# StarsX/RayTracedGGX

Hardware: AMD Instinct MI355X
Metric: Mrays/s + ms/frame, bunny 1920x1080 1spp+denoise, 1/2/4/8 GPUs (higher is better)
Workload: dtype f32; 1 GPU; configs[1]: bunny.obj + rnl_cross env, 1920x1080, 1spp GGX reflection + full denoise chain (refl H,V; diff H,V, shared-memory variant; temporal; tone map), all-metal default materials, dt=1/60; parallelism=row strips x1, history_apron_rows=18, history_overreach_rows=0, setup_priming_frames=256, trace_workgroup_waves=12

## Files before the change

### raytracedggx_amd/csrc/raytrace.hip

```cpp
#include <cstring>
#include "rt_queue.h"
#include "rt_traverse.h"

namespace rt {

#define RT_PI 3.1415926535897f
#define RT_SGPR(v) ((uint32_t)__builtin_amdgcn_readfirstlane((int)(v)))

struct EnvRef { const uint2* __restrict__ texels; uint32_t size, mips; const uint32_t* __restrict__ mipOffset; };

RT_DEV void cubeFaceUV(f3 d, int& face, float& u, float& v) {
  const float ax = fabsf(d.x), ay = fabsf(d.y), az = fabsf(d.z);
  if (ax >= ay && ax >= az) { face = d.x >= 0.0f ? 0 : 1; u = (d.x >= 0.0f ? -d.z : d.z) / ax; v = -d.y / ax; }
  else if (ay >= az) { face = d.y >= 0.0f ? 2 : 3; u = d.x / ay; v = (d.y >= 0.0f ? d.z : -d.z) / ay; }
  else { face = d.z >= 0.0f ? 4 : 5; u = (d.z >= 0.0f ? d.x : -d.x) / az; v = -d.y / az; }
}
RT_DEV f3 cubeFaceDir(int face, float u, float v) {
  switch (face) {
    case 0: return mk3(1.0f, -v, -u);
    case 1: return mk3(-1.0f, -v, u);
    case 2: return mk3(u, 1.0f, v);
    case 3: return mk3(u, -1.0f, -v);
    case 4: return mk3(u, -v, 1.0f);
    default: return mk3(-u, -v, -1.0f);
  }
}
template <bool MIP0 = false>
RT_DEV f3 cubeTexel(const EnvRef& e, uint32_t mip, int face, int x, int y) {
  const int s = (int)((e.size >> mip) ? (e.size >> mip) : 1u);
  if (x < 0 || y < 0 || x >= s || y >= s) {
    const float u = ((float)x + 0.5f) / (float)s * 2.0f - 1.0f, v = ((float)y + 0.5f) / (float)s * 2.0f - 1.0f;
    float uu, vv; cubeFaceUV(cubeFaceDir(face, u, v), face, uu, vv);
    x = (int)floorf((uu * 0.5f + 0.5f) * (float)s); y = (int)floorf((vv * 0.5f + 0.5f) * (float)s);
    x = min(max(x, 0), s - 1); y = min(max(y, 0), s - 1);
  }
  const uint2 t = e.texels[(MIP0 ? 0u : e.mipOffset[mip]) + (uint32_t)face * (uint32_t)(s * s) + (uint32_t)(y * s + x)];
  return mk3(f16ToF32(t.x & 0xFFFFu), f16ToF32(t.x >> 16), f16ToF32(t.y & 0xFFFFu));
}
template <bool MIP0 = false>
RT_DEV f3 cubeBilinear(const EnvRef& e, uint32_t mip, int face, float u, float v) {
  const int s = (int)((e.size >> mip) ? (e.size >> mip) : 1u);
  const float x = (u * 0.5f + 0.5f) * (float)s - 0.5f, y = (v * 0.5f + 0.5f) * (float)s - 0.5f;
  const float x0 = floorf(x), y0 = floorf(y);
  const float fx = x - x0, fy = y - y0;
  const int ix = (int)x0, iy = (int)y0;
  const float w00 = (1.0f - fx) * (1.0f - fy), w10 = fx * (1.0f - fy), w01 = (1.0f - fx) * fy, w11 = fx * fy;
  const f3 c00 = cubeTexel<MIP0>(e, mip, face, ix, iy), c10 = cubeTexel<MIP0>(e, mip, face, ix + 1, iy);
  const f3 c01 = cubeTexel<MIP0>(e, mip, face, ix, iy + 1), c11 = cubeTexel<MIP0>(e, mip, face, ix + 1, iy + 1);
  return ((c00 * w00 + c10 * w10) + c01 * w01) + c11 * w11;
}
RT_DEV f3 environmentLevel0(const EnvRef& e, f3 dir) {
  int face; float u, v; cubeFaceUV(dir, face, u, v);
  return cubeBilinear<true>(e, 0u, face, u, v);
}
__device__ __noinline__ f3 environment(EnvRef e, f3 dir, float level) {
  int face; float u, v; cubeFaceUV(dir, face, u, v);
  const float maxLevel = (float)(e.mips - 1);
  const float l = fminf(fmaxf(level, 0.0f), maxLevel);
  const float l0 = floorf(l), fl = l - l0;
  const uint32_t m0 = (uint32_t)l0, m1 = min(m0 + 1, e.mips - 1);
  const f3 a = cubeBilinear(e, m0, face, u, v);
  if (fl == 0.0f) return a;
  const f3 b = cubeBilinear(e, m1, face, u, v);
  return a * (1.0f - fl) + b * fl;
}

RT_DEV f3 evaluateSHIrradiance(const float* __restrict__ sh, f3 norm) {
  const float c1 = 0.42904276540489171563379376569857f, c2 = 0.51166335397324424423977581244463f;
  const float c3 = 0.24770795610037568833406429782001f, c4 = 0.88622692545275801364908374167057f;
  const float x = -norm.x, y = -norm.y, z = norm.z;
#define SHL(i) mk3(sh[3 * (i)], sh[3 * (i) + 1], sh[3 * (i) + 2])
  f3 irr = (c1 * (x * x - y * y)) * SHL(8);
  irr = irr + (c3 * (3.0f * z * z - 1.0f)) * SHL(6);
  irr = irr + c4 * SHL(0);
  irr = irr + (2.0f * c1) * ((SHL(4) * x * y + SHL(7) * x * z) + SHL(5) * y * z);
  irr = irr + (2.0f * c2) * ((SHL(3) * x + SHL(1) * y) + SHL(2) * z);
#undef SHL
  return mk3(fmaxf(0.0f, irr.x), fmaxf(0.0f, irr.y), fmaxf(0.0f, irr.z));
}

RT_DEV f2 getUV(f3 n, f3 p, f3 scl) {
  f2 uv; uv.x = fabsf(n.x) * p.y * scl.y; uv.y = fabsf(n.x) * p.z * scl.z;
  uv.x += fabsf(n.y) * p.z * scl.z; uv.y += fabsf(n.y) * p.x * scl.x;
  uv.x += fabsf(n.z) * p.x * scl.x; uv.y += fabsf(n.z) * p.y * scl.y;
  uv.x = uv.x * 0.5f + 0.5f; uv.y = uv.y * 0.5f + 0.5f;
  return uv;
}
RT_DEV f2 getRoughMetal(const RtggxCBMaterial& mat, uint32_t inst, f2 uv) {
  float rough = mat.RoughMetals[inst][0];
  if (inst == 0) {
    const uint32_t px = ftou(uv.x * 5.0f) & 1u, py = ftou(uv.y * 5.0f) & 1u;
    rough = (px ^ py) ? rough * 0.25f : rough;
  }
  f2 r; r.x = rough; r.y = mat.RoughMetals[inst][1];
  return r;
}

RT_DEV float visSmith(float roughness, float NoV, float NoL) {
  const float a = roughness * roughness, a2 = a * a;
  const float v = NoV + sqrtf(NoV * (NoV - NoV * a2) + a2);
  const float l = NoL + sqrtf(NoL * (NoL - NoL * a2) + a2);
  return 1.0f / (v * l);
}
RT_DEV f3 fSchlick(f3 spec, float VoH) {
  const float x = 1.0f - VoH, x2 = x * x;
  const float fc = (x2 * x2) * x;
  const float s = saturatef(50.0f * spec.y) * fc;
  return mk3(s + (1.0f - fc) * spec.x, s + (1.0f - fc) * spec.y, s + (1.0f - fc) * spec.z);
// ... 23 lines not shown
  const f3 xAxis = normalize3(cross3(up, n));
  const f3 yAxis = cross3(n, xAxis);
  return (xAxis * l.x + yAxis * l.y) + n * l.z;
}
RT_DEV f3 vndfHalfVector(f3 n, f3 v, float alpha, float cosPhi, float sinPhi, float u) {
  const f3 up = fabsf(n.y) < 0.999f ? mk3(0.0f, 1.0f, 0.0f) : mk3(1.0f, 0.0f, 0.0f);
  const f3 xAxis = normalize3(cross3(up, n));
  const f3 yAxis = cross3(n, xAxis);
  const f3 ve = mk3(dot3(v, xAxis), dot3(v, yAxis), dot3(v, n));
  const f3 vh = normalize3(mk3(alpha * ve.x, alpha * ve.y, ve.z));
  const float lensq = vh.x * vh.x + vh.y * vh.y;
  const f3 t1v = lensq > 0.0f ? mk3(-vh.y, vh.x, 0.0f) * (1.0f / sqrtf(lensq)) : mk3(1.0f, 0.0f, 0.0f);
  const f3 t2v = cross3(vh, t1v);
  const float r = sqrtf(u);
  const float t1 = r * cosPhi;
  float t2 = r * sinPhi;
  const float sw = 0.5f * (1.0f + vh.z);
  t2 = (1.0f - sw) * sqrtf(1.0f - t1 * t1) + sw * t2;
  const f3 nh = (t1 * t1v + t2 * t2v) + sqrtf(fmaxf(0.0f, (1.0f - t1 * t1) - t2 * t2)) * vh;
  const f3 hl = normalize3(mk3(alpha * nh.x, alpha * nh.y, fmaxf(0.0f, nh.z)));
  return (xAxis * hl.x + yAxis * hl.y) + n * hl.z;
}
RT_DEV f3 reflectionHalfVector(bool vndf, f3 N, f3 V, float a, float cosPhi, float sinPhi, float xiY) {
  if (vndf) return vndfHalfVector(N, V, a, cosPhi, sinPhi, xiY);
  const float cosTheta = sqrtf((1.0f - xiY) / (1.0f + (a * a - 1.0f) * xiY));
  const float sinTheta = sqrtf(1.0f - cosTheta * cosTheta);
  return localToWorld(N, mk3(cosPhi * sinTheta, sinPhi * sinTheta, cosTheta));
}
RT_DEV f3 reflectionWeight(bool vndf, f3 N, f3 V, f3 Hh, float NoL, f2 rghMtl, f3 color) {
  const float a = rghMtl.x * rghMtl.x;
  const f3 f0 = mk3(lerpf(0.04f, color.x, rghMtl.y), lerpf(0.04f, color.y, rghMtl.y), lerpf(0.04f, color.z, rghMtl.y));
  const float NoV = saturatef(dot3(N, V));
  const float VoH = saturatef(dot3(V, Hh));
  const f3 F = fSchlick(f0, VoH);
  const float vis = visSmith(rghMtl.x, NoV, NoL);
  const float NoH = saturatef(dot3(N, Hh));
  const float k = 4.0f * VoH / NoH;
  f3 w = mk3(((NoL * F.x) * vis) * k, ((NoL * F.y) * vis) * k, ((NoL * F.z) * vis) * k);
  if (vndf) {
    const float a2 = a * a;
    const float g1l = (2.0f * NoL) / (NoL + sqrtf(NoL * (NoL - NoL * a2) + a2));
    w = mk3(F.x * g1l, F.y * g1l, F.z * g1l);
  }
  return w;
}
RT_DEV f3 diffuseDirection(f3 N, float cosPhi, float sinPhi, float xiY) {
  const float cosTheta = 1.0f - 2.0f * xiY;
  const float sinTheta = sqrtf(1.0f - cosTheta * cosTheta);
  return normalize3(N + mk3(cosPhi * sinTheta, sinPhi * sinTheta, cosTheta));
}
struct Tri3 { f3 pos[3], nrm[3]; };
RT_DEV Tri3 getVertices(const float4* __restrict__ fat, uint32_t prim) {
  const float4* p = fat + 5 * (size_t)prim;
  const float4 a = p[0], b = p[1], c = p[2], d = p[3], e = p[4];
  Tri3 v;
  v.pos[0] = mk3(a.x, a.y, a.z); v.nrm[0] = mk3(a.w, b.x, b.y);
  v.pos[1] = mk3(b.z, b.w, c.x); v.nrm[1] = mk3(c.y, c.z, c.w);
  v.pos[2] = mk3(d.x, d.y, d.z); v.nrm[2] = mk3(d.w, e.x, e.y);
  return v;
}
struct Attrib { f3 Pos, Nrm; f2 UV; };
RT_DEV Attrib interpAttrib(const Tri3& v, float b1, float b2) {
  const float w0 = 1.0f - (b1 + b2);
  Attrib a;
  a.Pos = (w0 * v.pos[0] + b1 * v.pos[1]) + b2 * v.pos[2];
  a.Nrm = (w0 * v.nrm[0] + b1 * v.nrm[1]) + b2 * v.nrm[2];
  a.UV = getUV(a.Nrm, a.Pos, mk3(1.0f, 0.2f, 1.0f));
  return a;
}
RT_DEV f2 calcBarycentrics(const f4 p[3], f2 ndc) {
  const f3 invW = mk3(1.0f / p[0].w, 1.0f / p[1].w, 1.0f / p[2].w);
  f2 ndc0, ndc1, ndc2;
  ndc0.x = p[0].x * invW.x; ndc0.y = p[0].y * invW.x; ndc1.x = p[1].x * invW.y; ndc1.y = p[1].y * invW.y; ndc2.x = p[2].x * invW.z; ndc2.y = p[2].y * invW.z;
  const float det = (ndc2.x - ndc1.x) * (ndc0.y - ndc1.y) - (ndc2.y - ndc1.y) * (ndc0.x - ndc1.x);
  const float invDet = 1.0f / det;
  const f3 dPdx = mk3(ndc1.y - ndc2.y, ndc2.y - ndc0.y, ndc0.y - ndc1.y) * invDet;
  const f3 dPdy = mk3(ndc2.x - ndc1.x, ndc0.x - ndc2.x, ndc1.x - ndc0.x) * invDet;
  f2 dv; dv.x = ndc.x - ndc0.x; dv.y = ndc.y - ndc0.y;
  const float interpInvW = (invW.x + dv.x * dot3(invW, dPdx)) + dv.y * dot3(invW, dPdy);
  const float interpW = 1.0f / interpInvW;
  f2 b;
  b.x = interpW * (dv.x * dPdx.y * invW.y + dv.y * dPdy.y * invW.y);
  b.y = interpW * (dv.x * dPdx.z * invW.z + dv.y * dPdy.z * invW.z);
  return b;
}

struct GenArgs {
  const unsigned long long* visDepth; uint32_t* depthOut;
  unsigned long long* visNext; uint32_t* zeroNext0; uint32_t* zeroNext1;
  const uint32_t* visDirty; const uint32_t* visDirtyNext; uint32_t* visDirtyNextOut;
  const uint32_t* skyPrev; uint32_t* skyOut; uint32_t skyEpoch, skyPrevRun;
  uint32_t* normalOut; uint16_t* roughMetalOut; uint32_t* velocityOut; uint32_t* reflOut; uint32_t* diffOut;
  const uint16_t* roughMetalPrev;
  const uint32_t* diffPrev;
  const float4* fat0; const float4* fat1;
  const uint2* env; const uint32_t* envMipOffset; uint32_t envSize, envMips;
  const float* cosSin;
  RayRec* rays; HitKey* hits; uint32_t* binCount; uint32_t binSlots;
  uint32_t* frameRays;
  uint32_t tilesX, numTiles, rowBegin, rowEnd;
  uint32_t* binWork; uint32_t* splitList; uint32_t* splitCount; uint32_t splitWork, frontWork, splitMaxShift, splitCap;
};

RT_DEV void sampleParamWide(const FrameParams& fp, const float* table, uint32_t pixel, float& xiY, float& cosPhi, float& sinPhi) {
  uint32_t s = rng(pixel); s += fp.g.FrameIndex; s = rng(s); s &= fp.sampleMask;
  xiY = (float)(rng(s) & 0xffffu) / 65536.0f;
  const float2 cs = reinterpret_cast<const float2*>(table)[s];
// ... 25 lines not shown
  if (wantDiff && kD < A.binSlots) { dst[kD] = rd; keys[kD] = hitKey(RT_RAY_TMAX, 0xFFFFFFFFu); }
  if (threadIdx.x != 0) return;
  const uint32_t nRaysInBin = min(nR + nD, A.binSlots);
  uint32_t mark = 0u;
  if (A.binWork != nullptr) {
    const uint32_t w = A.binWork[bin];
    A.binWork[bin] = 0u;
    uint32_t shift = 0u;
    while (shift < A.splitMaxShift && (w >> shift) > A.splitWork) ++shift;
    const uint32_t n = (shift || w > A.frontWork) ? 1u << shift : 0u;
    if (n) {
      const uint32_t base = atomicAdd(A.splitCount, n);
      const bool fits = base + n <= A.splitCap;
      for (uint32_t k = 0; k < n && base + k < A.splitCap; ++k) A.splitList[base + k] = fits ? ((shift << 28) | (k << 24) | bin) : 0xFFFFFFFFu;
      mark = fits ? (shift << 1) | 1u : 0u;
    }
  }
  A.binCount[bin] = nRaysInBin | (mark << 8);
}
template <int RATE, bool WIDE = false>
__global__ void __launch_bounds__(256, RT_GEN_MIN_BLOCKS) rayGenKernel(const FrameParams* __restrict__ fpp, GenArgs A) {
  const FrameParams& fp = *fpp;
  if (blockIdx.x == 0) A.frameRays[threadIdx.x] = 0u;
  if (blockIdx.x == 0 && threadIdx.x == 0 && A.visNext != nullptr) { *A.zeroNext0 = 0u; *A.zeroNext1 = 0u; }
  uint32_t tile = blockIdx.x;
  if constexpr (RATE == 4) {
    const uint32_t superX = (A.tilesX + 1u) >> 1, sup = blockIdx.x >> 2;
    const uint32_t tx = (sup % superX) * 2u + (blockIdx.x & 1u), ty = (sup / superX) * 2u + ((blockIdx.x >> 1) & 1u);
    tile = ty * A.tilesX + tx;
    if (tx >= A.tilesX || tile >= A.numTiles) {
      if (threadIdx.x == 0) { A.binCount[blockIdx.x] = 0u; if (A.binWork != nullptr) A.binWork[blockIdx.x] = 0u; }
      return;
    }
  }
  const uint32_t wave = threadIdx.x >> 6, lane = threadIdx.x & 63u;
  const uint32_t px = (tile % A.tilesX) * 16 + (wave & 1u) * 8 + (lane & 7u);
  const uint32_t py = A.rowBegin + (tile / A.tilesX) * 16 + (wave >> 1) * 8 + (lane >> 3);
  const bool inside = px < fp.W && py < A.rowEnd;
  const bool traced = RATE == 1 || quadTraced(px, py, fp.g.FrameIndex);
  uint32_t wordHere, wordNext, skyWord;
  asm volatile("s_load_dword %0, %3, %6\n\ts_load_dword %1, %4, %6\n\ts_load_dword %2, %5, %6\n\ts_waitcnt lgkmcnt(0)"
               : "=&s"(wordHere), "=&s"(wordNext), "=&s"(skyWord) : "s"(A.visDirty), "s"(A.visDirtyNext), "s"(A.skyPrev), "s"(tile * 4u) : "memory");
  const bool drawn = wordHere != 0u;
  const bool clearNext = A.visNext != nullptr && wordNext != 0u;
  const uint32_t skyPrevRun = (skyWord >> 8) == A.skyEpoch ? skyWord & 0xFFu : 0u;
  const uint32_t skyWordOut = (A.skyEpoch << 8) | (drawn || RATE != 1 ? 0u : min(skyPrevRun + 1u, RT_SKY_RUN_CAP));
  if (RATE == 1 && !drawn && !clearNext && skyPrevRun >= A.skyPrevRun) {
    if (threadIdx.x == 0) A.skyOut[tile] = skyWordOut;
    return;
  }
  const EnvRef env{A.env, A.envSize, A.envMips, A.envMipOffset};
  bool wantRefl = false, wantDiff = false;
  RayRec rr, rd;
  if (inside) {
    const uint32_t W = fp.W, H = fp.H;
    const size_t pix = (size_t)py * W + px;
    const unsigned long long visWord = drawn ? A.visDepth[pix] : RT_VIS_CLEAR;
    if (clearNext) A.visNext[pix] = RT_VIS_CLEAR;
    float xiY = 0.0f, cosPhi = 0.0f, sinPhi = 0.0f;
    if constexpr (WIDE) { if (drawn) sampleParamWide(fp, A.cosSin, py * W + px, xiY, cosPhi, sinPhi); }
    else if (drawn) {
      uint32_t s = py * W + px;
      s = rng(s); s += fp.g.FrameIndex; s = rng(s); s %= 256u;
      xiY = (float)(rng(s) & 0xffffu) / 65536.0f;
      cosPhi = A.cosSin[s]; sinPhi = A.cosSin[256 + s];
    }
    uint32_t visibility = (uint32_t)visWord;
    A.depthOut[pix] = (uint32_t)(visWord >> 32);
    f2 screenPos; screenPos.x = ((float)px + 0.5f) / (float)W * 2.0f - 1.0f; screenPos.y = ((float)py + 0.5f) / (float)H * 2.0f - 1.0f;
    screenPos.y = -screenPos.y;
    const f3 eye = mk3(fp.rg.EyePt[0], fp.rg.EyePt[1], fp.rg.EyePt[2]);
    bool hit; f3 N, V, P, color; f2 rghMtl, velocity; uint32_t inst = 0, prim = 0;
    if (visibility > 0) {
      --visibility;
      hit = true; inst = visibility >> 24; prim = visibility & 0xFFFFFFu;
      asm volatile("" : "+v"(prim));
      const Tri3 v = getVertices(inst ? A.fat1 : A.fat0, prim);
      const M4 wvp = cbLoad4x4(fp.g.WorldViewProjs[inst]);
      f4 p[3];
      for (int k = 0; k < 3; ++k) p[k] = mulPoint(v.pos[k], wvp);
      screenPos.x -= fp.rg.ProjBias[0]; screenPos.y -= fp.rg.ProjBias[1];
      const f2 bary = calcBarycentrics(p, screenPos);
      const Attrib a = interpAttrib(v, bary.x, bary.y);
      color = mk3(fp.mat.BaseColors[inst][0], fp.mat.BaseColors[inst][1], fp.mat.BaseColors[inst][2]);
      rghMtl = getRoughMetal(fp.mat, inst, a.UV);
      const f4 hPrev = mulPoint(a.Pos, cbLoad4x4(fp.g.WorldViewProjsPrev[inst]));
      velocity.x = (screenPos.x - hPrev.x / hPrev.w) * 0.5f; velocity.y = (screenPos.y - hPrev.y / hPrev.w) * -0.5f;
      const f4 P4 = mulPoint(a.Pos, cbLoad4x3(fp.g.Worlds[inst]));
      P = mk3(P4.x, P4.y, P4.z);
      N = normalize3(mulDir(a.Nrm, cbLoad3x3(inst ? fp.g.WorldIT1 : fp.g.WorldITs0)));
      V = normalize3(eye - P);
    } else {
      f4 sp4; sp4.x = screenPos.x; sp4.y = screenPos.y; sp4.z = 0.0f; sp4.w = 1.0f;
      const f4 world = mulVec4(sp4, cbLoad4x4(fp.rg.ProjToWorld));
      hit = false; velocity.x = 0.0f; velocity.y = 0.0f;
      P = mk3(world.x / world.w, world.y / world.w, world.z / world.w);
      N = mk3(0.0f, 0.0f, 0.0f);
      V = normalize3(eye - P);
      rghMtl.x = 0.0f; rghMtl.y = 0.0f;
      color = mk3(0.0f, 0.0f, 0.0f);
    }
    A.normalOut[pix] = packR10G10B10A2(N.x * 0.5f + 0.5f, N.y * 0.5f + 0.5f, N.z * 0.5f + 0.5f, hit ? 1.0f : 0.0f);
    A.roughMetalOut[pix] = hit ? (uint16_t)packR8G8(rghMtl.x, rghMtl.y) : A.roughMetalPrev[pix];
    A.velocityOut[pix] = packR16G16F(velocity.x, velocity.y);

    if (!hit) {
      const uint32_t c = packR11G11B10F(environmentLevel0(env, -V));
      A.reflOut[pix] = c;
      A.diffOut[pix] = c;
    } else {
      const uint32_t skip = (inst << 24) | prim;
      if (traced) {
        const float a = rghMtl.x * rghMtl.x;
        const bool vndf = (fp.flags & RT_FLAG_VNDF) != 0u;
        f3 Hh;
        if (vndf) Hh = vndfHalfVector(N, V, a, cosPhi, sinPhi, xiY);
        else {
          const float cosTheta = sqrtf((1.0f - xiY) / (1.0f + (a * a - 1.0f) * xiY));
          const float sinTheta = sqrtf(1.0f - cosTheta * cosTheta);
          Hh = localToWorld(N, mk3(cosPhi * sinTheta, sinPhi * sinTheta, cosTheta));
        }
        const f3 R = reflect3(-V, Hh);
        const float NoL = dot3(N, R);
        if (NoL <= 0.0f) A.reflOut[pix] = 0u;
        else {
          const f3 f0 = mk3(lerpf(0.04f, color.x, rghMtl.y), lerpf(0.04f, color.y, rghMtl.y), lerpf(0.04f, color.z, rghMtl.y));
          const float NoV = saturatef(dot3(N, V));
          const float VoH = saturatef(dot3(V, Hh));
          const f3 F = fSchlick(f0, VoH);
          const float vis = visSmith(rghMtl.x, NoV, NoL);
          const float NoH = saturatef(dot3(N, Hh));
          const float k = 4.0f * VoH / NoH;
          wantRefl = true;
          rr.ox = P.x; rr.oy = P.y; rr.oz = P.z;
          rr.dx = R.x; rr.dy = R.y; rr.dz = R.z;
          rr.pixel = (uint32_t)pix; rr.skip = skip; rr.flags = 0u;
          rr.wx = ((NoL * F.x) * vis) * k; rr.wy = ((NoL * F.y) * vis) * k; rr.wz = ((NoL * F.z) * vis) * k;
          if (vndf) {
            const float a2 = a * a;
            const float g1l = (2.0f * NoL) / (NoL + sqrtf(NoL * (NoL - NoL * a2) + a2));
            rr.wx = F.x * g1l; rr.wy = F.y * g1l; rr.wz = F.z * g1l;
          }
        }
      }
      if (rghMtl.y < 1.0f) {
        if (traced) {
          const float cosTheta = 1.0f - 2.0f * xiY;
          const float sinTheta = sqrtf(1.0f - cosTheta * cosTheta);
          const f3 dir = normalize3(N + mk3(cosPhi * sinTheta, sinPhi * sinTheta, cosTheta));
          wantDiff = true;
          rd.ox = P.x; rd.oy = P.y; rd.oz = P.z;
          rd.dx = dir.x; rd.dy = dir.y; rd.dz = dir.z;
          rd.pixel = (uint32_t)pix; rd.skip = skip; rd.flags = 1u;
          rd.wx = color.x * (1.0f - 0.04f); rd.wy = color.y * (1.0f - 0.04f); rd.wz = color.z * (1.0f - 0.04f);
        }
      } else if (A.diffPrev != nullptr) A.diffOut[pix] = A.diffPrev[pix];
    }
  }
  if (threadIdx.x == 0) { A.skyOut[tile] = skyWordOut; if (clearNext) A.visDirtyNextOut[tile] = 0u; }
  if constexpr (RATE == 4) { rayGenQuadBin(A, wantRefl, wantDiff, rr, rd); return; }

  const uint32_t bin = blockIdx.x * 4u + wave;
  const unsigned long long maskR = __ballot(wantRefl), maskD = __ballot(wantDiff), below = (1ull << lane) - 1ull;
  const uint32_t nR = (uint32_t)__popcll(maskR);
  RayRec* dst = A.rays + (size_t)bin * A.binSlots;
  HitKey* keys = A.hits + (size_t)bin * A.binSlots;
  if (wantRefl) { const uint32_t k = (uint32_t)__popcll(maskR & below); dst[k] = rr; keys[k] = hitKey(RT_RAY_TMAX, 0xFFFFFFFFu); }
  const uint32_t kD = nR + (uint32_t)__popcll(maskD & below);
  if (wantDiff && kD < A.binSlots) { dst[kD] = rd; keys[kD] = hitKey(RT_RAY_TMAX, 0xFFFFFFFFu); }
  const uint32_t nRaysInBin = min(nR + (uint32_t)__popcll(maskD), A.binSlots);
  if (A.binWork == nullptr) {
    if (lane == 0) A.binCount[bin] = nRaysInBin;
    return;
  }
  __shared__ uint32_t want[4], listBase;
  uint32_t shift = 0u, n = 0u;
  if (lane == 0) {
    const uint32_t w = A.binWork[bin];
    A.binWork[bin] = 0u;
    while (shift < A.splitMaxShift && (w >> shift) > A.splitWork) ++shift;
    n = (shift || w > A.frontWork) ? 1u << shift : 0u;
    want[wave] = n;
  }
  __syncthreads();
  if (threadIdx.x == 0) { const uint32_t total = want[0] + want[1] + want[2] + want[3]; listBase = total ? atomicAdd(A.splitCount, total) : 0u; }
  __syncthreads();
  if (lane == 0) {
    uint32_t base = listBase, mark = 0u;
    for (uint32_t k = 0; k < wave; ++k) base += want[k];
    if (n) {
      const bool fits = base + n <= A.splitCap;
      for (uint32_t k = 0; k < n && base + k < A.splitCap; ++k) A.splitList[base + k] = fits ? ((shift << 28) | (k << 24) | bin) : 0xFFFFFFFFu;
      mark = fits ? (shift << 1) | 1u : 0u;
    }
    A.binCount[bin] = nRaysInBin | (mark << 8);
  }
}

struct ShadeArgs {
  const RayRec* rays; const HitKey* hits; const uint32_t* binCount; uint32_t binSlots;
  const float4* fat0; const float4* fat1;
  const uint2* env; const uint32_t* envMipOffset; uint32_t envSize, envMips;
  const float* sh;
  uint32_t* reflOut; uint32_t* diffOut;
  const uint32_t* diffPrev; const unsigned long long* visDepth; uint32_t tilesX, rowBegin, rowEnd, carryMask;
  const uint32_t* tileWords;
  RayRec* spawnRays; HitKey* spawnHits; uint32_t* spawnCount; const float* cosSin;
  float* accRefl; float* accDiff;
};

enum ShadePass { SHADE_FINAL = 0, SHADE_SPAWN = 1, SHADE_FINAL_DEEP = 2, SHADE_ACCUM = 3, SHADE_SPAWN_ACCUM = 4 };
constexpr bool shadeSpawns(int pass) { return pass == SHADE_SPAWN || pass == SHADE_SPAWN_ACCUM; }
constexpr bool shadeAccumulates(int pass) { return pass == SHADE_ACCUM || pass == SHADE_SPAWN_ACCUM; }

RT_DEV f3 reflectionDepth1(const EnvRef& env, f2 rghMtl, f3 N, f3 V, f3 color) {
  const float level = calcMipFromRoughness(rghMtl.x, (float)env.mips);
  const float a = rghMtl.x * rghMtl.x;
  const f3 R = reflect3(-V, N);
  const f3 dir = lerp3(N, R, (1.0f - a) * (sqrtf(1.0f - a) + a));
  const float NoL = dot3(N, dir);
  if (NoL <= 0.0f) return mk3(0.0f, 0.0f, 0.0f);
  const f3 e = environment(env, dir, level);
  const f3 f0 = mk3(lerpf(0.04f, color.x, rghMtl.y), lerpf(0.04f, color.y, rghMtl.y), lerpf(0.04f, color.z, rghMtl.y));
  const float NoV = saturatef(dot3(N, V));
  return e * envBRDFApprox(f0, rghMtl.x, NoV);
}

RT_DEV uint32_t quadTileWord(const uint32_t* words, uint32_t tile32, uint32_t tilesX, uint32_t tilesY) {
  const uint32_t superX = (tilesX + 1u) >> 1, tx = (tile32 % superX) * 2u, ty = (tile32 / superX) * 2u;
  const uint32_t i0 = ty * tilesX + tx;
  const bool right = tx + 1u < tilesX, down = ty + 1u < tilesY;
  const uint32_t i1 = right ? i0 + 1u : i0, i2 = down ? i0 + tilesX : i0, i3 = right && down ? i0 + tilesX + 1u : i0;
  uint32_t a, b, c, d;
  asm volatile("s_load_dword %0, %4, %5\n\ts_load_dword %1, %4, %6\n\ts_load_dword %2, %4, %7\n\ts_load_dword %3, %4, %8\n\ts_waitcnt lgkmcnt(0)"
               : "=&s"(a), "=&s"(b), "=&s"(c), "=&s"(d)
               : "s"(words), "s"(RT_SGPR(i0 * 4u)), "s"(RT_SGPR(i1 * 4u)), "s"(RT_SGPR(i2 * 4u)), "s"(RT_SGPR(i3 * 4u)) : "memory");
  return a | b | c | d;
}
template <int RATE, int PASS, bool WIDE = false>
__global__ void __launch_bounds__(256, RT_GEN_MIN_BLOCKS) shadeKernel(const FrameParams* __restrict__ fpp, ShadeArgs A) {
  const FrameParams& fp = *fpp;
  const EnvRef env{A.env, A.envSize, A.envMips, A.envMipOffset};
  const uint32_t tile = blockIdx.x;
  { uint32_t word;
    if constexpr (RATE == 1) asm volatile("s_load_dword %0, %1, %2\n\ts_waitcnt lgkmcnt(0)" : "=s"(word) : "s"(A.tileWords), "s"(tile * 4u) : "memory");
    else word = quadTileWord(A.tileWords, tile, A.tilesX, (A.rowEnd - A.rowBegin + 15u) / 16u);
    if (word == 0u) return; }
  const uint32_t bin = tile * 4u + (threadIdx.x >> 6);
  if (RATE == 1 && A.carryMask != 0u) {
    const uint32_t lane = threadIdx.x & 63u, wave = threadIdx.x >> 6;
    const uint32_t px = (tile % A.tilesX) * 16u + (wave & 1u) * 8u + (lane & 7u);
    const uint32_t py = A.rowBegin + (tile / A.tilesX) * 16u + (wave >> 1) * 8u + (lane >> 3);
    if (px < fp.W && py < A.rowEnd) {
      const size_t pix = (size_t)py * fp.W + px;
      const uint32_t vis = (uint32_t)A.visDepth[pix];
      if (vis != 0u && ((A.carryMask >> ((vis - 1u) >> 24)) & 1u)) A.diffOut[pix] = A.diffPrev[pix];
    }
  }
  const uint32_t count = min(A.binCount[bin] & 0xFFu, A.binSlots);
  uint32_t spawned = 0u;
  for (uint32_t i = threadIdx.x & 63u; i < count; i += 64u) {
    const size_t slot = (size_t)bin * A.binSlots + i;
    const float4* rp = reinterpret_cast<const float4*>(A.rays + slot);
    const float4 q0 = rp[0], q1 = rp[1], q2 = rp[2];
    const float4 ra = make_float4(q0.x, q0.y, q0.z, RT_RAY_TMIN), rb = make_float4(q0.w, q1.x, q1.y, RT_RAY_TMAX), rw = make_float4(q2.x, q2.y, q2.z, 0.0f);
    const uint4 rc = make_uint4(__float_as_uint(q1.z), __float_as_uint(q1.w), __float_as_uint(q2.w), 0u);
    const uint32_t hitId = hitKeyId(A.hits[slot]);
    const f3 dir = mk3(rb.x, rb.y, rb.z);
    const bool diffuseGroup = (rc.z & 1u) != 0u;
    const uint32_t srcInst = rc.y >> 24;
    f3 col;
    bool child = false; RayRec cr;
    if (hitId == 0xFFFFFFFFu) col = environmentLevel0(env, dir);
    else {
      const float m = fp.mat.RoughMetals[srcInst][1];
      const f3 preset = mk3(fp.mat.BaseColors[srcInst][0] * m, fp.mat.BaseColors[srcInst][1] * m, fp.mat.BaseColors[srcInst][2] * m);
      if (!diffuseGroup && preset.x <= 0.0f && preset.y <= 0.0f && preset.z <= 0.0f) col = preset;
      else {
        const uint32_t hInst = hitId >> 24;
        uint32_t hPrim = hitId & 0xFFFFFFu;
        asm volatile("" : "+v"(hPrim));
        const Tri3 v = getVertices(hInst ? A.fat1 : A.fat0, hPrim);
        float ht, hb1 = 0.0f, hb2 = 0.0f;
        woopTestVerts(toObject(ra.x, ra.y, ra.z, rb.x, rb.y, rb.z, hInst ? fp.invWorld[1] : fp.invWorld[0]), v.pos[0], v.pos[1], v.pos[2], ht, hb1, hb2);
        const Attrib a = interpAttrib(v, hb1, hb2);
        const f3 N = normalize3(mulDir(a.Nrm, cbLoad3x3(hInst ? fp.g.WorldIT1 : fp.g.WorldITs0)));
        const f2 rm = getRoughMetal(fp.mat, hInst, a.UV);
        f3 color = mk3(fp.mat.BaseColors[hInst][0], fp.mat.BaseColors[hInst][1], fp.mat.BaseColors[hInst][2]);
        const f3 V = -dir;
        if constexpr (!shadeSpawns(PASS)) {
          if (rm.y > 0.5f) col = reflectionDepth1(env, rm, N, V, color);
          else {
            if (diffuseGroup) color = color * (1.0f - rm.y);
            const f3 irr = evaluateSHIrradiance(A.sh, N);
            col = mk3(irr.x / RT_PI, irr.y / RT_PI, irr.z / RT_PI) * color;
          }
        } else {
          const f3 P = mk3(ra.x + ht * rb.x, ra.y + ht * rb.y, ra.z + ht * rb.z);
          float xiY, cosPhi, sinPhi;
          if constexpr (WIDE) sampleParamWide(fp, A.cosSin, rc.x, xiY, cosPhi, sinPhi);
          else {
            uint32_t s = rng(rc.x); s += fp.g.FrameIndex; s = rng(s); s %= 256u;
            xiY = (float)(rng(s) & 0xffffu) / 65536.0f; cosPhi = A.cosSin[s]; sinPhi = A.cosSin[256 + s];
          }
          const uint32_t toDiffImage = (rc.z ^ (rc.z >> 1)) & 1u;
          f3 w, L;
          if (rm.y > 0.5f) {
            const bool vndf = (fp.flags & RT_FLAG_VNDF) != 0u;
            const f3 Hh = reflectionHalfVector(vndf, N, V, rm.x * rm.x, cosPhi, sinPhi, xiY);
            L = reflect3(-V, Hh);
            const float NoL = dot3(N, L);
            if (NoL <= 0.0f) col = mk3(0.0f, 0.0f, 0.0f);
            else { w = reflectionWeight(vndf, N, V, Hh, NoL, rm, color); child = true; cr.flags = toDiffImage << 1; }
          } else {
            if (diffuseGroup) color = color * (1.0f - rm.y);
            L = diffuseDirection(N, cosPhi, sinPhi, xiY);
            w = color; child = true; cr.flags = 1u | ((toDiffImage ^ 1u) << 1);
          }
          if (child) {
            cr.ox = P.x; cr.oy = P.y; cr.oz = P.z; cr.dx = L.x; cr.dy = L.y; cr.dz = L.z;
            cr.pixel = rc.x; cr.skip = hitId;
            cr.wx = rw.x * w.x; cr.wy = rw.y * w.y; cr.wz = rw.z * w.z;
          }
        }
      }
    }
    if constexpr (shadeSpawns(PASS)) {
      const unsigned long long mask = __ballot(child);
      if (child) {
        const size_t k = (size_t)bin * A.binSlots + spawned + (uint32_t)__popcll(mask & ((1ull << (threadIdx.x & 63u)) - 1ull));
        A.spawnRays[k] = cr; A.spawnHits[k] = hitKey(RT_RAY_TMAX, 0xFFFFFFFFu);
      }
      spawned += (uint32_t)__popcll(mask);
      if (child) continue;
    }
    if constexpr (shadeAccumulates(PASS)) {
      float* acc = (((rc.z ^ (rc.z >> 1)) & 1u) != 0u ? A.accDiff : A.accRefl) + 3u * (size_t)rc.x;
      acc[0] = acc[0] + col.x * rw.x; acc[1] = acc[1] + col.y * rw.y; acc[2] = acc[2] + col.z * rw.z;
      continue;
    }
    const uint32_t packed = packR11G11B10F(mk3(col.x * rw.x, col.y * rw.y, col.z * rw.z));
// ... 503 lines not shown
```

### raytracedggx_amd/csrc/trace.hip

```cpp
#include <type_traits>
#include "rt_queue.h"
#include "rt_traverse.h"

namespace rt {

#define RT_PRIME_LAUNCHES 4u
#ifndef RT_STACK
#define RT_STACK 16
#endif

struct TraceArgs {
  const float4* nodes0; const float4* tris0;
  const float4* nodes1; const float4* tris1;
  int32_t root0, root1;
  uint32_t haveMesh0, haveMesh1;
  const RayRec* rays; HitKey* hits;
  const float2* tRange;
  const uint32_t* binCount; uint32_t numBins, binSlots;
  int32_t* overflow;
  uint32_t* rayTotals;
  uint32_t* stats;
  unsigned long long* runTotals;
  uint32_t countRowBegin, countRowEnd, width;
  size_t spillStride;
// ... 11 lines not shown
#endif
#ifndef RT_STEAL_ROUNDS
#define RT_STEAL_ROUNDS 2
#endif
#ifndef RT_LEAF_BATCH
#define RT_LEAF_BATCH 8u
#endif
#ifndef RT_PREFETCH
#define RT_PREFETCH 0
#endif
#define RT_SPILL_WAVES 16384u
#define RT_TOP_FIELDS 7
template <int WAVES, int TOP> struct TraceLds {
  int32_t stack[RT_STACK * 64 * WAVES];
  uint32_t victims[64 * WAVES];
  uint32_t next, done, pad[2];
  float4 top[TOP ? RT_TOP_FIELDS * RT_TOP_NODES : 1];
};
typedef __attribute__((address_space(3))) int32_t LdsInt;
typedef __attribute__((address_space(3))) uint32_t LdsUint;
typedef float __attribute__((ext_vector_type(4))) NativeFloat4;
typedef __attribute__((address_space(3))) NativeFloat4 LdsFloat4;
template <int TOP> __device__ __forceinline__ void traceItem(const FrameParams& fp, const TraceArgs& A, LdsInt* const stackMem, LdsUint* const victimMem, const LdsFloat4* const topMem, const uint32_t item, const uint32_t waveSlot) {
  const uint32_t lane = threadIdx.x & 63u;
  const uint32_t wave = (item >> 3) & 3u, vblock = ((item >> 5) << 3) | (item & 7u), ldsWave = threadIdx.x >> 6;
  uint32_t shift = A.sliceShift, bin, slice;
  if (vblock < A.splitBlocks) {
    const uint32_t item = vblock * 4u + wave;
    if (item >= min(*A.splitCount, A.splitBlocks * 4u)) return;
    const uint32_t e = A.splitList[item];
    if (e == 0xFFFFFFFFu) return;
    bin = e & 0xFFFFFFu; slice = (e >> 24) & 15u; shift = e >> 28;
    if (bin >= A.numBins) return;
  } else {
    const uint32_t slices = 1u << shift;
    const uint32_t blk = (vblock - A.splitBlocks) >> shift, sub = (vblock - A.splitBlocks) & (slices - 1u);
    uint32_t tile = blk;
    if (A.tilesX != 0u) {
      const uint32_t xcd = blk & 7u, local = blk >> 3;
      const uint32_t super = (local >> 6) * 8u + xcd, inSuper = local & 63u;
      const uint32_t superX = (A.tilesX + 7u) >> 3;
      const uint32_t tx = (super % superX) * 8u + (inSuper & 7u), ty = (super / superX) * 8u + (inSuper >> 3);
      if (tx >= A.tilesX || ty >= A.tilesY) return;
      tile = ty * A.tilesX + tx;
      uint32_t word;
      asm volatile("s_load_dword %0, %1, %2\n\ts_waitcnt lgkmcnt(0)" : "=s"(word) : "s"(A.tileWords), "s"(tile * 4u) : "memory");
      if (word == 0u) return;
    }
    bin = tile * 4u + ((sub * 4u + wave) >> shift); slice = (sub * 4u + wave) & (slices - 1u);
    if (bin >= A.numBins) return;
  }
  const uint32_t raysPerWave = 64u >> shift;
  const uint32_t countWord = A.binCount[bin];
  if (vblock >= A.splitBlocks && A.binWork != nullptr && (countWord >> 8) != 0u) return;
  const uint32_t count = min(countWord & 0xFFu, A.binSlots);
  if (count <= slice * raysPerWave) return;
  LdsInt* const stackBase = stackMem + ldsWave * (RT_STACK * 64);
  LdsInt* const stack = stackBase + lane;
  LdsUint* const victims = victimMem + ldsWave * 64;
  const size_t spillStride = A.spillStride;
  int32_t* const spill = A.overflow + (size_t)waveSlot * 64u + lane;
  const unsigned long long laneLt = (1ull << lane) - 1ull;
  uint32_t nRays = 0, work = 0;
#ifdef RT_TRACE_STATS
  uint32_t stNode = 0, stLeaf = 0, stIter = 0, stDeep = 0, stSteal = 0, stLeafPhase = 0;
  const unsigned long long stT0 = clock64(), stW0 = wall_clock64();
#endif
  for (uint32_t base = 0; base < count; base += 64u) {
  const uint32_t rayIndex = base + slice * raysPerWave + lane;
  const uint32_t slot = bin * A.binSlots + min(rayIndex, A.binSlots - 1u);
  const bool hasRay = lane < raysPerWave && rayIndex < count;

  const uint32_t raySlot = hasRay ? slot : bin * A.binSlots;
  const float4* rp = reinterpret_cast<const float4*>(A.rays + raySlot);
  const float4 q0 = rp[0], q1 = rp[1];
  const float4 ra = make_float4(q0.x, q0.y, q0.z, 0.0f), rb = make_float4(q0.w, q1.x, q1.y, 0.0f);
  const uint4 rc = make_uint4(__float_as_uint(q1.z), __float_as_uint(q1.w), 0u, 0u);
  float tmin0 = RT_RAY_TMIN, bestT = RT_RAY_TMAX;
  if (A.tRange != nullptr) { const float2 tr = A.tRange[raySlot]; tmin0 = tr.x; bestT = tr.y; }
  uint32_t bestId = 0xFFFFFFFFu;
  {
    const uint32_t row = rc.x / A.width;
    if (hasRay && row >= A.countRowBegin && row < A.countRowEnd) ++nRays;
  }

  auto traverse = [&](auto instTag) {
  constexpr uint32_t INST = decltype(instTag)::value;
  if ((INST ? A.haveMesh1 : A.haveMesh0) == 0u) return;
  const float4* const nodes = INST ? A.nodes1 : A.nodes0;
  const float4* const tris = INST ? A.tris1 : A.tris0;
  LaneRay r = toObject(ra.x, ra.y, ra.z, rb.x, rb.y, rb.z, fp.invWorld[INST]);
  float tmin = tmin0;
  uint32_t skip = rc.y;
  int32_t cur = (INST ? A.topCount1 : A.topCount0) ? RT_TOP_FLAG : (INST ? A.root1 : A.root0);
  int sp = 0, sb = 0;
  bool job = hasRay && bestT > tmin, helper = false;
  uint32_t owner = slot;
  float myT = bestT; uint32_t myId = bestId;

#if RT_PREFETCH
  float pf = 0.0f;
#endif
  for (;;) {
    const unsigned long long jobMask = __ballot(job);
    if (jobMask == 0ull) break;
    work += (uint32_t)__popcll(jobMask);
    if ((uint32_t)__popcll(~jobMask) >= RT_STEAL_MIN_IDLE) {
      for (int round = 0; round < RT_STEAL_ROUNDS; ++round) {
        const bool offers = job && sb < sp && sb < RT_STACK;
        const unsigned long long victimMask = __ballot(offers), idleMask = __ballot(!job);
        if (victimMask == 0ull || idleMask == 0ull) break;
        const uint32_t nv = (uint32_t)__popcll(victimMask), ni = (uint32_t)__popcll(idleMask);
        const uint32_t myV = (uint32_t)__popcll(victimMask & laneLt), myI = (uint32_t)__popcll(idleMask & laneLt);
        if (offers) victims[myV] = lane;
        const bool thief = !job && myI < nv;
        const uint32_t v = thief ? victims[myI] : lane;
        const int vsb = __shfl(sb, (int)v);
        const float v_ox = __shfl(r.ox, (int)v), v_oy = __shfl(r.oy, (int)v), v_oz = __shfl(r.oz, (int)v);
        const float v_ix = __shfl(r.ix, (int)v), v_iy = __shfl(r.iy, (int)v), v_iz = __shfl(r.iz, (int)v);
        const float v_Sx = __shfl(r.Sx, (int)v), v_Sy = __shfl(r.Sy, (int)v), v_Sz = __shfl(r.Sz, (int)v);
        const int v_kx = __shfl(r.kx, (int)v), v_ky = __shfl(r.ky, (int)v), v_kz = __shfl(r.kz, (int)v);
        const float v_tmin = __shfl(tmin, (int)v), v_bestT = __shfl(myT, (int)v);
        const uint32_t v_bestId = (uint32_t)__shfl((int)myId, (int)v), v_skip = (uint32_t)__shfl((int)skip, (int)v);
        const uint32_t v_owner = (uint32_t)__shfl((int)owner, (int)v);
        if (thief) {
          cur = stackBase[vsb * 64 + (int)v];
          r.ox = v_ox; r.oy = v_oy; r.oz = v_oz; r.ix = v_ix; r.iy = v_iy; r.iz = v_iz; r.Sx = v_Sx; r.Sy = v_Sy; r.Sz = v_Sz;
          r.kx = v_kx; r.ky = v_ky; r.kz = v_kz;
// ... 272 lines not shown
```

Before: 3168 Mrays/s.

## Stage frame constants in LDS and hoist per-pixel and ray loads ahead of dependencies

Result: no change. 3173 Mrays/s, median of 2 (+0.2%).

```diff
diff --git a/raytracedggx_amd/csrc/raytrace.hip b/raytracedggx_amd/csrc/raytrace.hip
--- a/raytracedggx_amd/csrc/raytrace.hip
+++ b/raytracedggx_amd/csrc/raytrace.hip
@@ -7,7 +7,19 @@
 #define RT_PI 3.1415926535897f
 #define RT_SGPR(v) ((uint32_t)__builtin_amdgcn_readfirstlane((int)(v)))
 
-struct EnvRef { const uint2* __restrict__ texels; uint32_t size, mips; const uint32_t* __restrict__ mipOffset; };
+RT_DEV void ldsCopy16(uint32_t* dst, const uint32_t* __restrict__ src) {
+  for (int k = 0; k < 16; ++k) dst[k] = src[k];
+}
+struct GenConsts { RtggxCBGlobal g; RtggxCBMaterial mat; };
+struct ShadeConsts { float invWorld[2][16]; float worldIT[32]; RtggxCBMaterial mat; uint32_t mipOffset[16]; };
+#define RT_WORLDIT_WORD0 80u
+static_assert(sizeof(RtggxCBGlobal) == 112 * 4 && sizeof(RtggxCBMaterial) == 16 * 4 && offsetof(RtggxCBGlobal, WorldITs0) == 88 * 4 && offsetof(RtggxCBGlobal, WorldIT1) == 100 * 4, "WorldIT1 follows WorldITs0; the LDS copies are made in 16-word pieces");
+
+typedef __attribute__((address_space(3))) uint32_t LdsWord;
+typedef uint32_t Words16 __attribute__((ext_vector_type(16)));
+template <class OFF> struct EnvRefT { const uint2* __restrict__ texels; uint32_t size, mips; OFF mipOffset; };
+typedef EnvRefT<const uint32_t* __restrict__> EnvRef;
+typedef EnvRefT<const LdsWord*> EnvRefLds;
 
 RT_DEV void cubeFaceUV(f3 d, int& face, float& u, float& v) {
   const float ax = fabsf(d.x), ay = fabsf(d.y), az = fabsf(d.z);
@@ -25,8 +37,8 @@
     default: return mk3(-u, -v, -1.0f);
   }
 }
-template <bool MIP0 = false>
-RT_DEV f3 cubeTexel(const EnvRef& e, uint32_t mip, int face, int x, int y) {
+template <bool MIP0 = false, class E>
+RT_DEV f3 cubeTexel(const E& e, uint32_t mip, int face, int x, int y) {
   const int s = (int)((e.size >> mip) ? (e.size >> mip) : 1u);
   if (x < 0 || y < 0 || x >= s || y >= s) {
     const float u = ((float)x + 0.5f) / (float)s * 2.0f - 1.0f, v = ((float)y + 0.5f) / (float)s * 2.0f - 1.0f;
@@ -37,8 +49,8 @@
   const uint2 t = e.texels[(MIP0 ? 0u : e.mipOffset[mip]) + (uint32_t)face * (uint32_t)(s * s) + (uint32_t)(y * s + x)];
   return mk3(f16ToF32(t.x & 0xFFFFu), f16ToF32(t.x >> 16), f16ToF32(t.y & 0xFFFFu));
 }
-template <bool MIP0 = false>
-RT_DEV f3 cubeBilinear(const EnvRef& e, uint32_t mip, int face, float u, float v) {
+template <bool MIP0 = false, class E>
+RT_DEV f3 cubeBilinear(const E& e, uint32_t mip, int face, float u, float v) {
   const int s = (int)((e.size >> mip) ? (e.size >> mip) : 1u);
   const float x = (u * 0.5f + 0.5f) * (float)s - 0.5f, y = (v * 0.5f + 0.5f) * (float)s - 0.5f;
   const float x0 = floorf(x), y0 = floorf(y);
@@ -49,11 +61,11 @@
   const f3 c01 = cubeTexel<MIP0>(e, mip, face, ix, iy + 1), c11 = cubeTexel<MIP0>(e, mip, face, ix + 1, iy + 1);
   return ((c00 * w00 + c10 * w10) + c01 * w01) + c11 * w11;
 }
-RT_DEV f3 environmentLevel0(const EnvRef& e, f3 dir) {
+template <class E> RT_DEV f3 environmentLevel0(const E& e, f3 dir) {
   int face; float u, v; cubeFaceUV(dir, face, u, v);
   return cubeBilinear<true>(e, 0u, face, u, v);
 }
-__device__ __noinline__ f3 environment(EnvRef e, f3 dir, float level) {
+template <class E> __device__ __noinline__ f3 environment(E e, f3 dir, float level) {
   int face; float u, v; cubeFaceUV(dir, face, u, v);
   const float maxLevel = (float)(e.mips - 1);
   const float l = fminf(fmaxf(level, 0.0f), maxLevel);
@@ -183,7 +195,8 @@
 struct Tri3 { f3 pos[3], nrm[3]; };
 RT_DEV Tri3 getVertices(const float4* __restrict__ fat, uint32_t prim) {
   const float4* p = fat + 5 * (size_t)prim;
-  const float4 a = p[0], b = p[1], c = p[2], d = p[3], e = p[4];
+  float4 a = p[0], b = p[1], c = p[2], d = p[3], e = p[4];
+  asm volatile("" : "+v"(e.x), "+v"(e.y));
   Tri3 v;
   v.pos[0] = mk3(a.x, a.y, a.z); v.nrm[0] = mk3(a.w, b.x, b.y);
   v.pos[1] = mk3(b.z, b.w, c.x); v.nrm[1] = mk3(c.y, c.z, c.w);
@@ -315,12 +328,14 @@
   const EnvRef env{A.env, A.envSize, A.envMips, A.envMipOffset};
   bool wantRefl = false, wantDiff = false;
   RayRec rr, rd;
+  const uint32_t W = fp.W, H = fp.H;
+  const size_t pix = (size_t)py * W + px;
+  unsigned long long visWord = RT_VIS_CLEAR;
+  float xiY = 0.0f, cosPhi = 0.0f, sinPhi = 0.0f;
+  uint16_t roughMetalCarry = 0; uint32_t diffCarry = 0u;
   if (inside) {
-    const uint32_t W = fp.W, H = fp.H;
-    const size_t pix = (size_t)py * W + px;
-    const unsigned long long visWord = drawn ? A.visDepth[pix] : RT_VIS_CLEAR;
+    if (drawn) visWord = A.visDepth[pix];
     if (clearNext) A.visNext[pix] = RT_VIS_CLEAR;
-    float xiY = 0.0f, cosPhi = 0.0f, sinPhi = 0.0f;
     if constexpr (WIDE) { if (drawn) sampleParamWide(fp, A.cosSin, py * W + px, xiY, cosPhi, sinPhi); }
     else if (drawn) {
       uint32_t s = py * W + px;
@@ -328,6 +343,24 @@
       xiY = (float)(rng(s) & 0xffffu) / 65536.0f;
       cosPhi = A.cosSin[s]; sinPhi = A.cosSin[256 + s];
     }
+    roughMetalCarry = A.roughMetalPrev[pix];
+    if (drawn && A.diffPrev != nullptr) diffCarry = A.diffPrev[pix];
+  }
+  uint32_t binCost = 0u;
+  if (RATE == 1 && A.binWork != nullptr)
+    asm volatile("s_load_dword %0, %1, %2\n\ts_waitcnt lgkmcnt(0)" : "=s"(binCost) : "s"(A.binWork), "s"(RT_SGPR((blockIdx.x * 4u + wave) * 4u)) : "memory");
+  __shared__ GenConsts tab;
+  if (lane == 0) {
+#pragma unroll 1
+    for (uint32_t part = 0; part < 2u; ++part) {
+      const uint32_t w = RT_SGPR(wave) * 32u + part * 16u;
+      constexpr uint32_t gWords = sizeof(RtggxCBGlobal) / 4u;
+      const uint32_t from = w < gWords ? (uint32_t)offsetof(FrameParams, g) / 4u + w : (uint32_t)offsetof(FrameParams, mat) / 4u + (w - gWords);
+      ldsCopy16(reinterpret_cast<uint32_t*>(&tab) + w, reinterpret_cast<const uint32_t*>(fpp) + from);
+    }
+  }
+  __syncthreads();
+  if (inside) {
     uint32_t visibility = (uint32_t)visWord;
     A.depthOut[pix] = (uint32_t)(visWord >> 32);
     f2 screenPos; screenPos.x = ((float)px + 0.5f) / (float)W * 2.0f - 1.0f; screenPos.y = ((float)py + 0.5f) / (float)H * 2.0f - 1.0f;
@@ -339,19 +372,19 @@
       hit = true; inst = visibility >> 24; prim = visibility & 0xFFFFFFu;
       asm volatile("" : "+v"(prim));
       const Tri3 v = getVertices(inst ? A.fat1 : A.fat0, prim);
-      const M4 wvp = cbLoad4x4(fp.g.WorldViewProjs[inst]);
+      const M4 wvp = cbLoad4x4(tab.g.WorldViewProjs[inst]);
       f4 p[3];
       for (int k = 0; k < 3; ++k) p[k] = mulPoint(v.pos[k], wvp);
       screenPos.x -= fp.rg.ProjBias[0]; screenPos.y -= fp.rg.ProjBias[1];
       const f2 bary = calcBarycentrics(p, screenPos);
       const Attrib a = interpAttrib(v, bary.x, bary.y);
-      color = mk3(fp.mat.BaseColors[inst][0], fp.mat.BaseColors[inst][1], fp.mat.BaseColors[inst][2]);
-      rghMtl = getRoughMetal(fp.mat, inst, a.UV);
-      const f4 hPrev = mulPoint(a.Pos, cbLoad4x4(fp.g.WorldViewProjsPrev[inst]));
+      color = mk3(tab.mat.BaseColors[inst][0], tab.mat.BaseColors[inst][1], tab.mat.BaseColors[inst][2]);
+      rghMtl = getRoughMetal(tab.mat, inst, a.UV);
+      const f4 hPrev = mulPoint(a.Pos, cbLoad4x4(tab.g.WorldViewProjsPrev[inst]));
       velocity.x = (screenPos.x - hPrev.x / hPrev.w) * 0.5f; velocity.y = (screenPos.y - hPrev.y / hPrev.w) * -0.5f;
-      const f4 P4 = mulPoint(a.Pos, cbLoad4x3(fp.g.Worlds[inst]));
+      const f4 P4 = mulPoint(a.Pos, cbLoad4x3(tab.g.Worlds[inst]));
       P = mk3(P4.x, P4.y, P4.z);
-      N = normalize3(mulDir(a.Nrm, cbLoad3x3(inst ? fp.g.WorldIT1 : fp.g.WorldITs0)));
+      N = normalize3(mulDir(a.Nrm, cbLoad3x3(tab.g.WorldITs0 + 12u * inst)));
       V = normalize3(eye - P);
     } else {
       f4 sp4; sp4.x = screenPos.x; sp4.y = screenPos.y; sp4.z = 0.0f; sp4.w = 1.0f;
@@ -364,7 +397,7 @@
       color = mk3(0.0f, 0.0f, 0.0f);
     }
     A.normalOut[pix] = packR10G10B10A2(N.x * 0.5f + 0.5f, N.y * 0.5f + 0.5f, N.z * 0.5f + 0.5f, hit ? 1.0f : 0.0f);
-    A.roughMetalOut[pix] = hit ? (uint16_t)packR8G8(rghMtl.x, rghMtl.y) : A.roughMetalPrev[pix];
+    A.roughMetalOut[pix] = hit ? (uint16_t)packR8G8(rghMtl.x, rghMtl.y) : roughMetalCarry;
     A.velocityOut[pix] = packR16G16F(velocity.x, velocity.y);
 
     if (!hit) {
@@ -417,7 +450,7 @@
           rd.pixel = (uint32_t)pix; rd.skip = skip; rd.flags = 1u;
           rd.wx = color.x * (1.0f - 0.04f); rd.wy = color.y * (1.0f - 0.04f); rd.wz = color.z * (1.0f - 0.04f);
         }
-      } else if (A.diffPrev != nullptr) A.diffOut[pix] = A.diffPrev[pix];
+      } else if (A.diffPrev != nullptr) A.diffOut[pix] = diffCarry;
     }
   }
   if (threadIdx.x == 0) { A.skyOut[tile] = skyWordOut; if (clearNext) A.visDirtyNextOut[tile] = 0u; }
@@ -439,7 +472,7 @@
   __shared__ uint32_t want[4], listBase;
   uint32_t shift = 0u, n = 0u;
   if (lane == 0) {
-    const uint32_t w = A.binWork[bin];
+    const uint32_t w = binCost;
     A.binWork[bin] = 0u;
     while (shift < A.splitMaxShift && (w >> shift) > A.splitWork) ++shift;
     n = (shift || w > A.frontWork) ? 1u << shift : 0u;
@@ -476,7 +509,7 @@
 constexpr bool shadeSpawns(int pass) { return pass == SHADE_SPAWN || pass == SHADE_SPAWN_ACCUM; }
 constexpr bool shadeAccumulates(int pass) { return pass == SHADE_ACCUM || pass == SHADE_SPAWN_ACCUM; }
 
-RT_DEV f3 reflectionDepth1(const EnvRef& env, f2 rghMtl, f3 N, f3 V, f3 color) {
+template <class E> RT_DEV f3 reflectionDepth1(const E& env, f2 rghMtl, f3 N, f3 V, f3 color) {
   const float level = calcMipFromRoughness(rghMtl.x, (float)env.mips);
   const float a = rghMtl.x * rghMtl.x;
   const f3 R = reflect3(-V, N);
@@ -503,13 +536,15 @@
 template <int RATE, int PASS, bool WIDE = false>
 __global__ void __launch_bounds__(256, RT_GEN_MIN_BLOCKS) shadeKernel(const FrameParams* __restrict__ fpp, ShadeArgs A) {
   const FrameParams& fp = *fpp;
-  const EnvRef env{A.env, A.envSize, A.envMips, A.envMipOffset};
   const uint32_t tile = blockIdx.x;
   { uint32_t word;
     if constexpr (RATE == 1) asm volatile("s_load_dword %0, %1, %2\n\ts_waitcnt lgkmcnt(0)" : "=s"(word) : "s"(A.tileWords), "s"(tile * 4u) : "memory");
     else word = quadTileWord(A.tileWords, tile, A.tilesX, (A.rowEnd - A.rowBegin + 15u) / 16u);
     if (word == 0u) return; }
   const uint32_t bin = tile * 4u + (threadIdx.x >> 6);
+  __shared__ ShadeConsts tab;
+  const float* const worldIT0 = tab.worldIT + (offsetof(RtggxCBGlobal, WorldITs0) / 4u - RT_WORLDIT_WORD0);
+  const EnvRefLds env{A.env, A.envSize, A.envMips, (const LdsWord*)tab.mipOffset};
   if (RATE == 1 && A.carryMask != 0u) {
     const uint32_t lane = threadIdx.x & 63u, wave = threadIdx.x >> 6;
     const uint32_t px = (tile % A.tilesX) * 16u + (wave & 1u) * 8u + (lane & 7u);
@@ -520,15 +555,40 @@
       if (vis != 0u && ((A.carryMask >> ((vis - 1u) >> 24)) & 1u)) A.diffOut[pix] = A.diffPrev[pix];
     }
   }
-  const uint32_t count = min(A.binCount[bin] & 0xFFu, A.binSlots);
+  const uint32_t countWord = A.binCount[bin];
+  uint32_t count = 0u;
   uint32_t spawned = 0u;
-  for (uint32_t i = threadIdx.x & 63u; i < count; i += 64u) {
-    const size_t slot = (size_t)bin * A.binSlots + i;
+  for (uint32_t base = 0u; base == 0u || base < count; base += 64u) {
+    const uint32_t i = base + (threadIdx.x & 63u);
+    const size_t slot = (size_t)bin * A.binSlots + min(i, A.binSlots - 1u);
     const float4* rp = reinterpret_cast<const float4*>(A.rays + slot);
     const float4 q0 = rp[0], q1 = rp[1], q2 = rp[2];
+    const HitKey key = A.hits[slot];
+    if (base == 0u) {
+      if ((threadIdx.x & 63u) == 0u) {
+        const uint32_t* const words = reinterpret_cast<const uint32_t*>(fpp);
+        uint32_t* const dst = reinterpret_cast<uint32_t*>(&tab);
+        switch (RT_SGPR(threadIdx.x >> 6)) {
+          case 0: ldsCopy16(dst, words + offsetof(FrameParams, invWorld) / 4u); ldsCopy16(dst + 16, words + offsetof(FrameParams, invWorld) / 4u + 16u); break;
+          case 1: ldsCopy16(dst + 32, words + offsetof(FrameParams, g) / 4u + RT_WORLDIT_WORD0); ldsCopy16(dst + 48, words + offsetof(FrameParams, g) / 4u + RT_WORLDIT_WORD0 + 16u); break;
+          case 2: {
+            ldsCopy16(dst + 64, words + offsetof(FrameParams, mat) / 4u);
+            Words16 m;
+            asm volatile("s_load_dwordx16 %0, %1, 0x0\n\ts_waitcnt lgkmcnt(0)" : "=s"(m) : "s"(A.envMipOffset) : "memory");
+            for (int k = 0; k < 16; ++k) dst[80 + k] = m[k];
+            break; }
+          default: break;
+        }
+      }
+      __syncthreads();
+      uint32_t word = countWord;
+      asm volatile("" : "+v"(word));
+      count = RT_SGPR(min(word & 0xFFu, A.binSlots));
+    }
+    if (i >= count) continue;
     const float4 ra = make_float4(q0.x, q0.y, q0.z, RT_RAY_TMIN), rb = make_float4(q0.w, q1.x, q1.y, RT_RAY_TMAX), rw = make_float4(q2.x, q2.y, q2.z, 0.0f);
     const uint4 rc = make_uint4(__float_as_uint(q1.z), __float_as_uint(q1.w), __float_as_uint(q2.w), 0u);
-    const uint32_t hitId = hitKeyId(A.hits[slot]);
+    const uint32_t hitId = hitKeyId(key);
     const f3 dir = mk3(rb.x, rb.y, rb.z);
     const bool diffuseGroup = (rc.z & 1u) != 0u;
     const uint32_t srcInst = rc.y >> 24;
@@ -536,8 +596,8 @@
     bool child = false; RayRec cr;
     if (hitId == 0xFFFFFFFFu) col = environmentLevel0(env, dir);
     else {
-      const float m = fp.mat.RoughMetals[srcInst][1];
-      const f3 preset = mk3(fp.mat.BaseColors[srcInst][0] * m, fp.mat.BaseColors[srcInst][1] * m, fp.mat.BaseColors[srcInst][2] * m);
+      const float m = tab.mat.RoughMetals[srcInst][1];
+      const f3 preset = mk3(tab.mat.BaseColors[srcInst][0] * m, tab.mat.BaseColors[srcInst][1] * m, tab.mat.BaseColors[srcInst][2] * m);
       if (!diffuseGroup && preset.x <= 0.0f && preset.y <= 0.0f && preset.z <= 0.0f) col = preset;
       else {
         const uint32_t hInst = hitId >> 24;
@@ -545,11 +605,11 @@
         asm volatile("" : "+v"(hPrim));
         const Tri3 v = getVertices(hInst ? A.fat1 : A.fat0, hPrim);
         float ht, hb1 = 0.0f, hb2 = 0.0f;
-        woopTestVerts(toObject(ra.x, ra.y, ra.z, rb.x, rb.y, rb.z, hInst ? fp.invWorld[1] : fp.invWorld[0]), v.pos[0], v.pos[1], v.pos[2], ht, hb1, hb2);
+        woopTestVerts(toObject(ra.x, ra.y, ra.z, rb.x, rb.y, rb.z, tab.invWorld[hInst]), v.pos[0], v.pos[1], v.pos[2], ht, hb1, hb2);
         const Attrib a = interpAttrib(v, hb1, hb2);
-        const f3 N = normalize3(mulDir(a.Nrm, cbLoad3x3(hInst ? fp.g.WorldIT1 : fp.g.WorldITs0)));
-        const f2 rm = getRoughMetal(fp.mat, hInst, a.UV);
-        f3 color = mk3(fp.mat.BaseColors[hInst][0], fp.mat.BaseColors[hInst][1], fp.mat.BaseColors[hInst][2]);
+        const f3 N = normalize3(mulDir(a.Nrm, cbLoad3x3(worldIT0 + 12u * hInst)));
+        const f2 rm = getRoughMetal(tab.mat, hInst, a.UV);
+        f3 color = mk3(tab.mat.BaseColors[hInst][0], tab.mat.BaseColors[hInst][1], tab.mat.BaseColors[hInst][2]);
         const f3 V = -dir;
         if constexpr (!shadeSpawns(PASS)) {
           if (rm.y > 0.5f) col = reflectionDepth1(env, rm, N, V, color);
diff --git a/raytracedggx_amd/csrc/trace.hip b/raytracedggx_amd/csrc/trace.hip
--- a/raytracedggx_amd/csrc/trace.hip
+++ b/raytracedggx_amd/csrc/trace.hip
@@ -87,6 +87,9 @@
   }
   const uint32_t raysPerWave = 64u >> shift;
   const uint32_t countWord = A.binCount[bin];
+  const uint32_t slotAhead = bin * A.binSlots + min(slice * raysPerWave + lane, A.binSlots - 1u);
+  NativeFloat4 q0 = reinterpret_cast<const NativeFloat4*>(A.rays + slotAhead)[0], q1 = reinterpret_cast<const NativeFloat4*>(A.rays + slotAhead)[1];
+  asm volatile("" : "+v"(q0), "+v"(q1));
   if (vblock >= A.splitBlocks && A.binWork != nullptr && (countWord >> 8) != 0u) return;
   const uint32_t count = min(countWord & 0xFFu, A.binSlots);
   if (count <= slice * raysPerWave) return;
@@ -107,8 +110,10 @@
   const bool hasRay = lane < raysPerWave && rayIndex < count;
 
   const uint32_t raySlot = hasRay ? slot : bin * A.binSlots;
-  const float4* rp = reinterpret_cast<const float4*>(A.rays + raySlot);
-  const float4 q0 = rp[0], q1 = rp[1];
+  if (base != 0u) {
+    const NativeFloat4* rp = reinterpret_cast<const NativeFloat4*>(A.rays + raySlot);
+    q0 = rp[0]; q1 = rp[1];
+  }
   const float4 ra = make_float4(q0.x, q0.y, q0.z, 0.0f), rb = make_float4(q0.w, q1.x, q1.y, 0.0f);
   const uint4 rc = make_uint4(__float_as_uint(q1.z), __float_as_uint(q1.w), 0u, 0u);
   float tmin0 = RT_RAY_TMIN, bestT = RT_RAY_TMAX;
```
